# jmg049/Spectrograms

Hardware: AMD Instinct MI355X
Metric: STFT frames/sec (f32, n_fft=1024 hop=256) (higher is better)
Workload: dtype f32

## Files before the change

### spectrograms_amd/csrc/kernels_r32x16.hip

```cpp
#include <type_traits>
#include <utility>

#include "binaural_kind.h"
#include "buffer_ops.h"
#include "fft_inreg.h"
#include "r32x16_layout.h"
#include "sgx_internal.h"

namespace sgx {
namespace {

using namespace inreg;
using namespace r32x16;

typedef int v4i __attribute__((ext_vector_type(4)));
typedef int v2i __attribute__((ext_vector_type(2)));

__device__ __forceinline__ float db_f32(float x) { return __builtin_log2f(x) * 3.01029995663981195f; }

template <int AMP>
__device__ __forceinline__ float amp_f32(float p, float eps) {
    if constexpr (AMP == AMP_MAGNITUDE) return sqrtf(p);
    else if constexpr (AMP == AMP_DB) return db_f32(fmaxf(p, eps));
    else return p;
}
__device__ __forceinline__ float power_of(v2f x) { return __builtin_fmaf(x.x, x.x, x.y * x.y); }

__device__ __forceinline__ unsigned lds_addr(const void *p) { return (unsigned)(size_t)p; }

#ifdef SGX_STAMPS
__device__ unsigned long long g_stamps[32];
#define SGX_STAMP(i)                                                                        \
    do {                                                                                    \
        unsigned long long t_;                                                              \
        __builtin_amdgcn_sched_barrier(0);                                                  \
        asm volatile("s_memtime %0\n\ts_waitcnt lgkmcnt(0)" : "=s"(t_)::"memory");          \
        __builtin_amdgcn_sched_barrier(0);                                                  \
        st_acc[i] += t_ - st_prev;                                                          \
        st_prev = t_;                                                                       \
    } while (0)
#define SGX_STAMP_PARAMS , unsigned long long *st_acc, unsigned long long &st_prev
#define SGX_STAMP_ARGS , st_acc, st_prev
#else
#define SGX_STAMP(i)
#define SGX_STAMP_PARAMS
#define SGX_STAMP_ARGS
#endif

#ifndef SGX_BANDSEG
#define SGX_BANDSEG 0
#endif
#ifndef SGX_BANDTRIP
#define SGX_BANDTRIP 0
#endif
#ifndef SGX_BANDFMA
#define SGX_BANDFMA 0
#endif
#ifndef SGX_BANDPF
#define SGX_BANDPF 0
#endif
#ifndef SGX_ODDHOP
#define SGX_ODDHOP 1
#endif
#ifndef SGX_DMA
#define SGX_DMA 0
#endif
#ifndef SGX_ONEPATH
#define SGX_ONEPATH 1
#endif

template <int OFF>
__device__ __forceinline__ void ds_read64(v2f &d, unsigned addr) {
    asm volatile("ds_read_b64 %0, %1 offset:%2" : "=v"(d) : "v"(addr), "n"(OFF));
}
template <int OFF>
__device__ __forceinline__ void ds_read128(v4f &d, unsigned addr) {
    asm volatile("ds_read_b128 %0, %1 offset:%2" : "=v"(d) : "v"(addr), "n"(OFF));
}
template <int N>
__device__ __forceinline__ void tie8(v2f *d) {
    if constexpr (N >= 0)
        asm volatile("s_waitcnt lgkmcnt(%8)"
                     : "+v"(d[0]), "+v"(d[1]), "+v"(d[2]), "+v"(d[3]), "+v"(d[4]), "+v"(d[5]), "+v"(d[6]), "+v"(d[7])
                     : "n"(N));
    else
        asm volatile("" : "+v"(d[0]), "+v"(d[1]), "+v"(d[2]), "+v"(d[3]), "+v"(d[4]), "+v"(d[5]), "+v"(d[6]), "+v"(d[7]));
}
template <int N>
__device__ __forceinline__ void tie16(v2f (&d)[16]) {
    tie8<N>(&d[0]);
    tie8<-1>(&d[8]);
}
template <bool XSPAD, int N1>
constexpr int col_off() { return N1 * 128 + (XSPAD ? (N1 >> 3) * 128 : 0); }
template <bool XSPAD, int PAR, int... K>
__device__ __forceinline__ void read_cols(v2f (&x)[16], v2f (&w)[16], unsigned xaddr, unsigned waddr, std::integer_sequence<int, K...>) {
    ((ds_read64<col_off<XSPAD, 2 * K + PAR>()>(x[K], xaddr), ds_read64<(2 * K + PAR) * 128>(w[K], waddr)), ...);
}

template <int HOP>
constexpr int p512_off_a(int n1) { return 64 * n1 + (64 * n1 / (8 * HOP)) * 64; }
template <int HOP>
constexpr int p512_off_b(int n1) { return 64 * n1 + 4 * HOP + ((64 * n1 + 4 * HOP) / (8 * HOP)) * 64; }
template <int O0, int O1>
__device__ __forceinline__ void ds_read2x32(v2f &d, unsigned addr) {
    static_assert(O0 >= 0 && O0 < 256 && O1 >= 0 && O1 < 256, "ds_read2_b32: 8-bit dword offsets");
    asm volatile("ds_read2_b32 %0, %1 offset0:%2 offset1:%3" : "=v"(d) : "v"(addr), "n"(O0), "n"(O1));
}
template <int HOP, int PAR, int... K>
__device__ __forceinline__ void read_cols512(v2f (&x)[16], v2f (&w)[16], const unsigned (&base)[8], unsigned waddr, std::integer_sequence<int, K...>) {
    ((ds_read2x32<(p512_off_a<HOP>(2 * K + PAR) - p512_off_a<HOP>((2 * K + PAR) & ~3)) / 4, (p512_off_b<HOP>(2 * K + PAR) - p512_off_a<HOP>((2 * K + PAR) & ~3)) / 4>(
          x[K], base[(2 * K + PAR) >> 2]),
      ds_read64<(2 * K + PAR) * 128>(w[K], waddr)),
     ...);
}

template <int PAR, int... K>
__device__ __forceinline__ void read_cols_odd(v2f (&x)[16], v2f (&w)[16], const unsigned (&base)[4], unsigned waddr, std::integer_sequence<int, K...>) {
    ((ds_read2x32<((2 * K + PAR) & 7) * 32, ((2 * K + PAR) & 7) * 32 + 1>(x[K], base[(2 * K + PAR) >> 3]), ds_read64<(2 * K + PAR) * 128>(w[K], waddr)), ...);
}

template <int PAR, int... K>
__device__ __forceinline__ void read_win(v2f (&w)[16], unsigned waddr, std::integer_sequence<int, K...>) {
    (ds_read64<(2 * K + PAR) * 128>(w[K], waddr), ...);
}

template <int OFF>
__device__ __forceinline__ void dma16_to_lds(__amdgpu_buffer_rsrc_t r, int voff, unsigned lds_base) {
    unsigned keep;
    asm volatile("s_mov_b32 %0, m0\n\ts_mov_b32 m0, %3\n\ts_nop 0\n\tbuffer_load_dwordx4 %1, %2, 0 offen offset:%4 lds\n\ts_mov_b32 m0, %0"
                 : "=&s"(keep)
                 : "v"(voff), "s"(r), "s"(lds_base), "n"(OFF)
                 : "memory");
}
template <bool XSPAD, int R, int ROUNDS>
__device__ __forceinline__ void dma_rounds(__amdgpu_buffer_rsrc_t r, int voff, unsigned xs_base, unsigned wave) {
    if constexpr (R < ROUNDS) {
        const unsigned c0 = R * 256u + wave * 64u;
        dma16_to_lds<0>(r, voff + R * 4096, xs_base + c0 * 16u + (XSPAD ? (c0 >> 6) * 128u : 0u));
        dma_rounds<XSPAD, R + 1, ROUNDS>(r, voff, xs_base, wave);
    }
}

template <bool CONJ>
__device__ __forceinline__ v2f cmul_reg(v2f x, v2f t) {
    const v2f c = x * lo2(t);
    v2f r;
    if constexpr (CONJ) asm("v_pk_fma_f32 %0, %1, %2, %3 op_sel:[1,1,0] op_sel_hi:[0,1,1] neg_hi:[0,1,0]" : "=v"(r) : "v"(x), "v"(t), "v"(c));
    else asm("v_pk_fma_f32 %0, %1, %2, %3 op_sel:[1,1,0] op_sel_hi:[0,1,1] neg_lo:[0,1,0]" : "=v"(r) : "v"(x), "v"(t), "v"(c));
    return r;
}
__device__ __forceinline__ v2f split_tw(v2f D, v2f w) {
    const v2f c = lo2(D) * w;
    v2f r;
    asm("v_pk_fma_f32 %0, %1, %2, %3 op_sel:[1,1,0] op_sel_hi:[1,0,1] neg_lo:[0,1,0]" : "=v"(r) : "v"(D), "v"(w), "v"(c));
    return r;
}

__device__ __forceinline__ void load_tw1(const StftArgs &a, unsigned n2, v2f (&twa)[4], v2f (&twb)[8]) {
    const v2f *t1 = (const v2f *)a.tw1 + n2;
#pragma unroll
    for (int q = 0; q < 4; ++q) twa[q] = t1[16 * 8 * q];
#pragma unroll
    for (int q = 0; q < 8; ++q) twb[q] = t1[16 * q];
}

template <bool P2>
__device__ __forceinline__ void twiddle_store(v2f (&xr)[32], const v2f (&twa)[4], const v2f (&twb)[8], unsigned char *dst) {
#pragma unroll
    for (int k1 = 0; k1 < 32; ++k1) {
        const int qa = k1 >> 3, qb = k1 & 7;
        v2f r = xr[k1];
        if constexpr (P2) {
            if (k1 == 0) r = cmul_reg<true>(r, twa[2]);
        } else {
            if (qb) r = cmulv(r, twb[qb]);
            if (qa) r = cmulv(r, twa[qa]);
        }
#if defined(SGX_ABL_NOEXW)
        asm volatile("" ::"v"(r), "v"(dst));
#elif defined(SGX_ABL_ADDTID)
        asm volatile("ds_write_addtid_b32 %0 offset:%2\n\tds_write_addtid_b32 %1 offset:%3" ::"v"(r.x), "v"(r.y), "n"(k1 * 512), "n"(k1 * 512 + 256) : "memory");
#else
        *(v2f *)(dst + k1 * 128) = r;
#endif
    }
}

__device__ __forceinline__ void read_rows(const unsigned char *exf, unsigned ra, unsigned rb, v2f (&A)[16], v2f (&B)[16]) {
    const v4f *pa = (const v4f *)(exf + ra * 128);
    const v4f *pb = (const v4f *)(exf + rb * 128);
#pragma unroll
    for (int c = 0; c < 8; ++c) {
        const v4f q = pa[c];
        A[2 * c] = (v2f){q.x, q.y};
        A[2 * c + 1] = (v2f){q.z, q.w};
    }
#pragma unroll
    for (int c = 0; c < 8; ++c) {
        const v4f q = pb[c];
        B[2 * c] = (v2f){q.x, q.y};
        B[2 * c + 1] = (v2f){q.z, q.w};
    }
}

struct JobOfs {
    unsigned a1, b1, a2, b2, mid;
};
__device__ __forceinline__ JobOfs job_offsets(unsigned j, unsigned n_frames) {
    const unsigned c1 = j == 0 ? 16u : j, c2 = j == 0 ? 0u : j + 256u;
    return JobOfs{c1 * n_frames, (512u - 224u - c1) * n_frames, c2 * n_frames, (512u - 224u - c2) * n_frames, 256u * n_frames};
}

__device__ __forceinline__ void pass2_twiddle(v2f (&A)[16], v2f (&B)[16], const v2f (&t)[16]) {
#pragma unroll
    for (int n = 1; n < 16; ++n) {
        A[n] = cmul_reg<false>(A[n], t[n]);
        B[n] = cmul_reg<true>(B[n], t[n]);
    }
}

struct PwAddr {
    float *up, *down;
};
template <int MODE, int AMP, bool PWT, bool ROT>
__device__ __forceinline__ void pass2_compute(v2f (&A)[16], v2f (&B)[16], bool j0, float eps, const v4f *tw, __amdgpu_buffer_rsrc_t ro,
                                              unsigned oa1, unsigned ob1, unsigned oa2, unsigned ob2, unsigned omid, unsigned step,
                                              float *pw_c1, float *pw_m1, float *pw_c2, float *pw_m2, float *pw_mid SGX_STAMP_PARAMS) {
    constexpr int R = ROT ? 1 : 0;
    Fft<16, false>::run(A, A);
    Fft<16, false>::run(B, B);
    const v2f a8 = ROT ? B[9] : A[8];
    if (j0) {
        if constexpr (ROT) {
            v2f nA[8], nB[16];
#pragma unroll
            for (int t = 0; t < 8; ++t) nA[t] = B[t + 1];
#pragma unroll
            for (int i = 0; i < 8; ++i) nB[(16 - i) & 15] = A[15 - i];
#pragma unroll
            for (int t = 0; t < 8; ++t) nB[8 - t] = B[(17 - t) & 15];
#pragma unroll
            for (int t = 0; t < 8; ++t) A[8 + t] = nA[t];
#pragma unroll
            for (int i = 0; i < 16; ++i) B[i] = nB[i];
        } else {
            v2f nA[16], nB[8];
#pragma unroll
            for (int i = 0; i < 8; ++i) { nA[i] = B[i]; nA[8 + i] = A[i]; }
            nB[7] = A[0];
#pragma unroll
            for (int t = 1; t < 8; ++t) nB[7 - t] = A[16 - t];
#pragma unroll
            for (int i = 0; i < 16; ++i) A[i] = nA[i];
#pragma unroll
            for (int i = 0; i < 8; ++i) B[i] = nB[i];
        }
        asm volatile("" ::: "memory");
    }
    SGX_STAMP(9);
    constexpr int PSTEP = MODE == OUT_BINAURAL ? 32 * 16 * 2 : PWT ? 32 * 16 : 32;
    auto emit = [&](unsigned voff, unsigned soff, float *pwp, v2f X, bool conj) {
#ifdef SGX_ABL_NOSTORE
        asm volatile("" ::"v"(X), "v"(voff));
        return;
#endif
        if constexpr (MODE == OUT_COMPLEX) {
            const v2f V = conj ? (v2f){X.x, -X.y} : X;
            __builtin_amdgcn_raw_buffer_store_b64(__builtin_bit_cast(v2i, V), ro, (int)voff, (int)soff, 0);
        } else if constexpr (MODE == OUT_MEL) {
#ifdef SGX_ABL_NOPW
            asm volatile("" ::"v"(X), "v"(pwp));
            return;
#endif
            *pwp = AMP == AMP_MAG_IN ? sqrtf(power_of(X)) : power_of(X);
        } else if constexpr (MODE == OUT_BINAURAL) {
            *(v2f *)pwp = conj ? (v2f){X.x, -X.y} : X;
        } else {
            __builtin_amdgcn_raw_buffer_store_b32(__builtin_bit_cast(int, amp_f32<AMP>(power_of(X), eps)), ro, (int)voff, (int)soff, 0);
        }
    };
    auto twi = [&](int i) {
        const v4f q = tw[i >> 1];
        return (i & 1) ? (v2f){q.z, q.w} : (v2f){q.x, q.y};
    };
    auto split = [&](v2f P, v2f Q, v2f w, v2f &X, v2f &Y) {
        const v2f E = pfma(Q, (v2f){1.f, -1.f}, P);
        const v2f D = pfma(Q, (v2f){-1.f, 1.f}, P);
        const v2f T = split_tw(D, w);
        X = E + T;
        Y = E - T;
    };
#pragma unroll
    for (int i = 0; i < 8; ++i) {
        v2f X, Y;
        split(A[i], B[(15 + R - i) & 15], twi(i), X, Y);
        emit(oa1, i * step, pw_c1 + i * PSTEP, X, false);
        emit(ob1, (7 - i) * step, pw_m1 + (7 - i) * PSTEP, Y, true);
    }
#pragma unroll
    for (int t = 0; t < 8; ++t) {
        v2f X, Y;
        split(A[8 + t], B[7 + R - t], twi(8 + t), X, Y);
        emit(oa2, t * step, pw_c2 + t * PSTEP, X, false);
        emit(ob2, (7 - t) * step, pw_m2 + (7 - t) * PSTEP, Y, true);
    }
    if (j0) emit(omid, 0u, pw_mid, a8 * (v2f){2.f, -2.f}, false);
    SGX_STAMP(10);
}

constexpr unsigned kP512Step = 16u * 64u;
template <int MODE, int AMP, bool PACK = false>
__device__ __forceinline__ void pass2_pair512(v2f (&A)[16], v2f (&B)[16], bool j0, float eps, __amdgpu_buffer_rsrc_t ro, unsigned vfull1,
                                              unsigned vhalf1, unsigned vfull2, unsigned vhalf2, unsigned vfullm, unsigned vhalfm, unsigned step,
                                              float *pw1, float *pw2, float *pwm) {
    Fft<16, false>::run(A, A);
    Fft<16, false>::run(B, B);
    const v2f a8 = A[8];
    if (j0) {
        v2f nA[16], nB[8];
#pragma unroll
        for (int i = 0; i < 8; ++i) { nA[i] = B[i]; nA[8 + i] = A[i]; }
        nB[7] = A[0];
#pragma unroll
        for (int t = 1; t < 8; ++t) nB[7 - t] = A[16 - t];
#pragma unroll
        for (int i = 0; i < 16; ++i) A[i] = nA[i];
#pragma unroll
        for (int i = 0; i < 8; ++i) B[i] = nB[i];
        asm volatile("" ::: "memory");
    }
    auto emit = [&](unsigned vfull, unsigned vhalf, int soff, v2f Xa, v2f Xb, bool conj, float *pwp) {
        if constexpr (MODE == OUT_MEL) {
            const float pa = power_of(Xa), pb = power_of(Xb);
            *(v2f *)pwp = AMP == AMP_MAG_IN ? (v2f){sqrtf(pa), sqrtf(pb)} : (v2f){pa, pb};
        } else if constexpr (MODE == OUT_COMPLEX) {
            const float sg = conj ? -1.f : 1.f;
            const v4f V = (v4f){Xa.x, sg * Xa.y, Xb.x, sg * Xb.y};
            if constexpr (PACK) {
                __builtin_amdgcn_raw_buffer_store_b64(__builtin_bit_cast(v2i, (v2f){V.x, V.y}), ro, (int)vfull, soff, 0);
                __builtin_amdgcn_raw_buffer_store_b64(__builtin_bit_cast(v2i, (v2f){V.z, V.w}), ro, (int)vhalf, soff, 0);
            } else {
                __builtin_amdgcn_raw_buffer_store_b128(__builtin_bit_cast(v4i, V), ro, (int)vfull + soff, 0, 0);
                __builtin_amdgcn_raw_buffer_store_b64(__builtin_bit_cast(v2i, (v2f){V.x, V.y}), ro, (int)vhalf, soff, 0);
            }
        } else {
            const v2f V = (v2f){amp_f32<AMP>(power_of(Xa), eps), amp_f32<AMP>(power_of(Xb), eps)};
            if constexpr (PACK) {
                const float va = V.x, vb = V.y;
                __builtin_amdgcn_raw_buffer_store_b32(__builtin_bit_cast(int, va), ro, (int)vfull, soff, 0);
                __builtin_amdgcn_raw_buffer_store_b32(__builtin_bit_cast(int, vb), ro, (int)vhalf, soff, 0);
            } else {
                __builtin_amdgcn_raw_buffer_store_b64(__builtin_bit_cast(v2i, V), ro, (int)vfull, soff, 0);
                __builtin_amdgcn_raw_buffer_store_b32(__builtin_bit_cast(int, V.x), ro, (int)vhalf, soff, 0);
            }
        }
    };
    auto pair = [&](v2f P, v2f Q, v2f &Xa, v2f &Xb) {
        Xa = pfma(Q, (v2f){1.f, -1.f}, P);
        const v2f D = pfma(Q, (v2f){-1.f, 1.f}, P);
        Xb = (v2f){D.y, -D.x};
    };
#pragma unroll
    for (int i = 0; i < 8; ++i) {
        v2f Xa, Xb;
        pair(A[i], B[15 - i], Xa, Xb);
        emit(vfull1, vhalf1, i * (int)step, Xa, Xb, false, pw1 + i * kP512Step);
    }
#pragma unroll
    for (int t = 0; t < 8; ++t) {
        v2f Xa, Xb;
        pair(A[8 + t], B[7 - t], Xa, Xb);
        if (j0) emit(vfull2 + t * step, vhalf2 + t * step, 0, Xa, Xb, false, pw2 + t * kP512Step);
        else emit(vfull2 + (7 - t) * step, vhalf2 + (7 - t) * step, 0, Xa, Xb, true, pw2 + (7 - t) * kP512Step);
    }
    if (j0) emit(vfullm, vhalfm, 0, (v2f){2.f * a8.x, 0.f}, (v2f){2.f * a8.y, 0.f}, false, pwm);
}

template <int AMP>
__device__ __forceinline__ void mel_tile_csr(const StftArgs &a, const float *pwall, unsigned b, unsigned f0, unsigned nf,
                                             float eps, unsigned t, unsigned nthreads) {
    const float *val = (const float *)a.mel_val;
    float *o = (float *)a.out + ((size_t)b * a.n_out) * a.n_frames + f0;
    for (unsigned idx = t; idx < 16u * a.n_mels; idx += nthreads) {
        const unsigned ff = idx & 15u, mm = idx >> 4;
        float acc = 0.0f;
// ... 233 lines not shown
    }
}

template <int STEPS>
constexpr int mfcc_row() { return (STEPS / 4) % 2 ? STEPS : STEPS + 4; }
template <int STEPS>
__device__ __forceinline__ void mfcc_tile(const StftArgs &a, const float *mq, const float *frag, unsigned mt, unsigned b, unsigned f0, unsigned nf,
                                          unsigned lane) {
    static_assert(STEPS % 4 == 0, "chain lengths are whole 16-byte reads");
    constexpr int RL = mfcc_row<STEPS>();
    const unsigned n = lane & 15u, q = lane >> 4;
    const bool mine = mt < a.mfcc_mtiles;
    v4acc acc = {0.f, 0.f, 0.f, 0.f};
    if (mine) {
        const v4f *pa = (const v4f *)(frag + ((size_t)mt * 64u + lane) * RL);
        const v4f *pb = (const v4f *)(mq + (q * 16u + n) * RL);
        v4f wa[STEPS / 4], vb[STEPS / 4];
#pragma unroll
        for (int g = 0; g < STEPS / 4; ++g) { wa[g] = pa[g]; vb[g] = pb[g]; }
#pragma unroll
        for (int g = 0; g < STEPS / 4; ++g) {
            acc = __builtin_amdgcn_mfma_f32_16x16x4f32(wa[g].x, vb[g].x, acc, 0, 0, 0);
            acc = __builtin_amdgcn_mfma_f32_16x16x4f32(wa[g].y, vb[g].y, acc, 0, 0, 0);
            acc = __builtin_amdgcn_mfma_f32_16x16x4f32(wa[g].z, vb[g].z, acc, 0, 0, 0);
            acc = __builtin_amdgcn_mfma_f32_16x16x4f32(wa[g].w, vb[g].w, acc, 0, 0, 0);
        }
    }
    const float *lift = frag + (size_t)a.mfcc_mtiles * 64u * RL;
    constexpr unsigned kDrop = 0x80000000u;
    const unsigned rows = a.n_mfcc - a.mfcc_skip;
    const unsigned obytes = (rows * a.n_frames - f0) * 4u;
    const __amdgpu_buffer_rsrc_t ro = make_rsrc((const float *)a.out + (size_t)b * rows * a.n_frames + f0, obytes);
    const unsigned mtr = mine ? mt : 0u;
#pragma unroll
    for (int r = 0; r < 4; ++r) {
        const unsigned c = 16u * mtr + 4u * q + r;
        const bool ok = mine && c >= a.mfcc_skip && c < a.n_mfcc && n < nf;
        __builtin_amdgcn_raw_buffer_store_b32(__builtin_bit_cast(int, acc[r] * lift[min(c, a.n_mfcc - 1u)]), ro,
                                              (int)(ok ? ((c - a.mfcc_skip) * a.n_frames + n) * 4u : kDrop), 0, 0);
    }
}

__host__ __device__ constexpr unsigned pwt512_index(unsigned k, unsigned f) { return (k >> 1) * 64u + (f >> 1) * 4u + (k & 1u) * 2u + (f & 1u); }
template <int AMP>
__device__ __forceinline__ void mel_tile_sched512(const StftArgs &a, const float *pwT, const unsigned *sched, unsigned b, unsigned f0,
                                                  unsigned nf, float eps, unsigned tid) {
    const unsigned wave = __builtin_amdgcn_readfirstlane(tid >> 6), lane = tid & 63u, slot = lane >> 4, fp = lane & 15u;
    const unsigned obytes = (a.n_out * a.n_frames - f0) * 4u;
    const __amdgpu_buffer_rsrc_t ro = make_rsrc((const float *)a.out + (size_t)b * a.n_out * a.n_frames + f0, obytes);
    constexpr unsigned kDrop = 0x80000000u;
    const unsigned fo0 = 2u * fp < nf ? 8u * fp : kDrop, fo1 = 2u * fp + 1u < nf ? 8u * fp + 4u : kDrop;
    const uint4 *info = (const uint4 *)(sched + kSchedHdr) + wave * 8u + slot;
    uint4 ca = info[0], cb = info[4];
#pragma unroll
    for (unsigned seg = 0; seg < (unsigned)kSchedSegs; ++seg) {
        const uint4 na = info[(seg + 1u) * 32u], nb = info[(seg + 1u) * 32u + 4u];
        const unsigned L = __builtin_amdgcn_readfirstlane(ca.x);
        const v4f *wa = (const v4f *)((const float *)sched + ca.y), *wb = (const v4f *)((const float *)sched + cb.y);
        const v4f *pa = (const v4f *)(pwT + (ca.z >> 1) * 64u) + fp, *pb = (const v4f *)(pwT + (cb.z >> 1) * 64u) + fp;
        v2f acca = {0.0f, 0.0f}, accb = {0.0f, 0.0f};
        for (unsigned t = 0; t < L; t += 4u) {
            const v4f w4a = wa[t >> 2], a0 = pa[(t >> 1) * 16u], a1 = pa[(t >> 1) * 16u + 16u];
            const v4f w4b = wb[t >> 2], b0 = pb[(t >> 1) * 16u], b1 = pb[(t >> 1) * 16u + 16u];
            acca = mul_add_unfused(w4a.x, (v2f){a0.x, a0.y}, acca);
            accb = mul_add_unfused(w4b.x, (v2f){b0.x, b0.y}, accb);
            acca = mul_add_unfused(w4a.y, (v2f){a0.z, a0.w}, acca);
            accb = mul_add_unfused(w4b.y, (v2f){b0.z, b0.w}, accb);
            acca = mul_add_unfused(w4a.z, (v2f){a1.x, a1.y}, acca);
            accb = mul_add_unfused(w4b.z, (v2f){b1.x, b1.y}, accb);
            acca = mul_add_unfused(w4a.w, (v2f){a1.z, a1.w}, acca);
            accb = mul_add_unfused(w4b.w, (v2f){b1.z, b1.w}, accb);
        }
        const bool ha = ca.w != 0xffffffffu, hb = cb.w != 0xffffffffu;
        const unsigned boa = ca.w * a.n_frames * 4u, bob = cb.w * a.n_frames * 4u;
        __builtin_amdgcn_raw_buffer_store_b32(__builtin_bit_cast(int, amp_f32<AMP>(acca.x, eps)), ro, (int)((ha && fo0 != kDrop) ? boa + fo0 : kDrop), 0, 0);
        __builtin_amdgcn_raw_buffer_store_b32(__builtin_bit_cast(int, amp_f32<AMP>(acca.y, eps)), ro, (int)((ha && fo1 != kDrop) ? boa + fo1 : kDrop), 0, 0);
        __builtin_amdgcn_raw_buffer_store_b32(__builtin_bit_cast(int, amp_f32<AMP>(accb.x, eps)), ro, (int)((hb && fo0 != kDrop) ? bob + fo0 : kDrop), 0, 0);
        __builtin_amdgcn_raw_buffer_store_b32(__builtin_bit_cast(int, amp_f32<AMP>(accb.y, eps)), ro, (int)((hb && fo1 != kDrop) ? bob + fo1 : kDrop), 0, 0);
        ca = na;
        cb = nb;
    }
}

template <int KIND>
__device__ __forceinline__ void binaural_tile(const StftArgs &a, const unsigned char *smem_all, unsigned b, unsigned f0, unsigned nf) {
    binaural::KindConst<float> c;
    c.pi = 3.14159265358979323846f;
    c.two_pi = 2.0f * c.pi;
    c.bw = (float)a.bin_bw;
    c.power = a.bin_power;
    c.wrapped = a.bin_wrapped;
    const v2f *L = (const v2f *)smem_all, *R = (const v2f *)(smem_all + kExBytes);
    float *out = (float *)a.out + ((size_t)b * a.bin_count) * a.n_frames + f0;
    for (unsigned i = threadIdx.x; i < a.bin_count * 16u; i += 512u) {
        const unsigned r = i >> 4, f = i & 15u, k = a.bin_start + r;
        const v2f l = L[k * 16u + f], q = R[k * 16u + f];
        const float v = binaural::binaural_value<float, KIND>(l.x, l.y, q.x, q.y, k, c);
        if (f < nf) out[(size_t)r * a.n_frames + f] = v;
    }
}

template <int MODE, int AMP, int ROUNDS, bool WIDE, bool XSPAD, bool PWT, int HOP512 = 0, bool PACK = false, int MSTEPS = 0>
__global__ __launch_bounds__(512, 2) void k_r32x16(StftArgs a, unsigned per_xcd, unsigned total, unsigned slots) {
    constexpr bool MFCC = MSTEPS != 0;
    static_assert(!MFCC || (PWT && AMP == AMP_DB && HOP512 == 0 && !PACK), "fused MFCC epilogue: Mel-dB on the schedule, n_fft 1024, one-signal tiles");
    constexpr bool P512 = HOP512 != 0;
    constexpr bool BIN = MODE == OUT_BINAURAL;
    static_assert(!BIN || (!WIDE && !PWT && !P512 && !PACK && !MFCC), "binaural: one-signal n_fft 1024 tiles, per-half pass 2");
    constexpr unsigned HS = BIN ? 1u : 2u;
    static_assert(!PACK || (ROUNDS == 0 && !WIDE && !XSPAD && (HOP512 == 0 ? (MODE != OUT_MEL || PWT) : MODE != OUT_MEL)),
                  "PACK: direct loads, one-half tiles; n_fft 1024: scheduled band stage, n_fft 512: per-bin outputs");
    constexpr unsigned SS512 = 8u * HOP512;
    static_assert(!P512 || PACK || (HOP512 % 4 == 0 && ROUNDS * 256 * 4 >= 31 * HOP512 + 512), "P512: 16-byte chunks, the whole tile staged");
    static_assert(!WIDE || MODE != OUT_MEL, "wide pass 2 needs a per-bin output");
    static_assert(!PWT || MODE == OUT_MEL, "PWT is a filterbank layout");
    static_assert(!P512 || (!WIDE && !XSPAD && (ROUNDS > 0 || PACK) && (PWT == (MODE == OUT_MEL))), "P512: staged samples (PACK: per-lane loads), scheduled band stage");
    constexpr bool DMA = SGX_DMA != 0 && PWT && ROUNDS > 0 && !P512;
    constexpr unsigned FPT = P512 ? 32u : 16u;
    constexpr unsigned NB = P512 ? 257u : 513u;
    extern __shared__ __attribute__((aligned(16))) unsigned char smem_all[];
    const unsigned half = __builtin_amdgcn_readfirstlane(threadIdx.x >> 8);
    const unsigned tid = threadIdx.x & 255u;
    constexpr bool H256M = HOP512 == 256 && MODE == OUT_MEL && !PACK;
    constexpr unsigned EXB = H256M ? (unsigned)kExBytesH256 : (unsigned)kExBytes, POFF = H256M ? (unsigned)kOutOffH256 : (unsigned)kOutOff;
    unsigned char *smem = smem_all + half * EXB;
    unsigned char *tabs = smem_all + 2 * EXB;
    if (threadIdx.x < 256u) ((v4f *)(tabs + kWinOff))[threadIdx.x] = ((const v4f *)a.window)[threadIdx.x];
    if (threadIdx.x < 256u) {
        const unsigned jj = threadIdx.x >> 4, ii = threadIdx.x & 15u;
        const v4f q = ((const v4f *)a.tw2)[jj * 17u + ii];
        *(v2f *)(tabs + kTw2Off + jj * kTw2Stride + ii * 8u) = (v2f){q.x, q.y};
        *(v2f *)(tabs + kTrOff + jj * 128u + ii * 8u) = ((const v2f *)a.tw1)[(jj == 0u ? 16u : jj) * 16u + ii];
    }
    unsigned *sched = (unsigned *)(tabs + kMelOff);
    if constexpr (PWT)
        for (unsigned i = threadIdx.x; i < a.mel_sched_words; i += 512u) sched[i] = a.mel_sched[i];
    float *mfrag = (float *)(tabs + kMelOff) + ((a.mel_sched_words + 3u) & ~3u);
    if constexpr (MFCC)
        for (unsigned i = threadIdx.x; i < a.mfcc_frag_words; i += 512u) mfrag[i] = ((const float *)a.mfcc_frag)[i];

    const unsigned xcd = blockIdx.x & 7u, slot = blockIdx.x >> 3;
    const unsigned lo = xcd * per_xcd;
    const unsigned hi = min(lo + per_xcd, total);
    unsigned wid = lo + slot * HS + (BIN ? 0u : half);
    unsigned lead = lo + slot * HS;

    const unsigned p1f = tid >> 4, n2 = tid & 15u;
    const unsigned lane = tid & 63u;
    const unsigned wv_ = WIDE ? threadIdx.x >> 6 : tid >> 6;
    const unsigned jq = WIDE ? lane >> 5 : lane >> 4, p2f = WIDE ? lane & 31u : lane & 15u;
    const unsigned j = wv_ + (WIDE ? 8u : 4u) * jq;
    constexpr bool TWP2 = !P512 && MODE != OUT_MEL;
    constexpr bool TRLDS = TWP2 && ROUNDS == 0 && !WIDE;
    const unsigned ra = j == 0 ? (TWP2 ? 16u : 0u) : j, rb = j == 0 ? (TWP2 ? 0u : 16u) : 32u - j;
    const float eps = (float)a.eps;
    constexpr unsigned ES = MODE == OUT_COMPLEX ? 8u : 4u;
    const JobOfs jo = job_offsets(j, a.n_frames);
    const unsigned step = 32u * a.n_frames * ES;
    const v4f *twj = (const v4f *)(tabs + kTw2Off + j * kTw2Stride);
    v2f twa[4], twb[8], tr[16];
    if constexpr (!TWP2) {
        load_tw1(a, n2, twa, twb);
    } else {
        twa[2] = ((const v2f *)a.tw1)[16 * 16 + n2];
        if constexpr (!TRLDS)
#pragma unroll
            for (int q = 0; q < 16; ++q) tr[q] = ((const v2f *)a.tw1)[ra * 16u + q];
    }

    constexpr int NCR = ROUNDS > 0 ? ROUNDS : 1;
    v4f creg[NCR];
    v2f xd[ROUNDS > 0 ? 1 : 32];
    const unsigned chunks = XSPAD ? 1216u : P512 ? (31u * HOP512 + 512u + 3u) >> 2 : (15u * a.hop + 1024u + 3u) >> 2;
    const unsigned hop = XSPAD ? 256u : (P512 && !PACK) ? (unsigned)HOP512 : a.hop;
    const unsigned row_bytes = (unsigned)a.n_samples * 4u;
    auto load_tile = [&](unsigned w) {
        const unsigned b = w / a.tiles, tile = w - b * a.tiles;
        const unsigned f0 = tile * FPT;
        const __amdgpu_buffer_rsrc_t rx = make_rsrc((const float *)(BIN && half ? a.x2 : a.x) + (size_t)b * a.sample_stride, row_bytes);
        const int tile_lo = (int)(f0 * hop) - (int)a.pad;
        const bool interior = tile_lo >= 0 && (unsigned)tile_lo + (FPT - 1u) * hop + (P512 ? 512u : 1024u) <= (unsigned)a.n_samples;
        if constexpr (ROUNDS > 0) {
#ifdef SGX_ABL_NOGLOAD
            for (int r = 0; r < ROUNDS; ++r) creg[r] = (v4f){(float)w, 1.f, 2.f, (float)r};
            return;
#endif
            const int vo = (tile_lo + 4 * (int)tid) * 4;
            if constexpr (DMA) {
                dma_rounds<XSPAD, 0, ROUNDS>(rx, vo, lds_addr(smem), __builtin_amdgcn_readfirstlane(tid >> 6));
                return;
            }
            if (SGX_ONEPATH || interior || P512) {
#pragma unroll
                for (int r = 0; r < ROUNDS; ++r)
                    if (SGX_ONEPATH || XSPAD || P512 || r * 256u + tid < chunks) creg[r] = __builtin_bit_cast(v4f, __builtin_amdgcn_raw_buffer_load_b128(rx, vo + r * 4096, 0, 0));
            } else {
#pragma unroll
                for (int r = 0; r < ROUNDS; ++r) {
                    v4i c;
#pragma unroll
                    for (int e = 0; e < 4; ++e) c[e] = __builtin_amdgcn_raw_buffer_load_b32(rx, vo + r * 4096 + 4 * e, 0, 0);
                    creg[r] = __builtin_bit_cast(v4f, c);
                }
            }
        } else if constexpr (PACK && P512) {
            const __amdgpu_buffer_rsrc_t rall = make_rsrc(a.x, a.x_bytes);
            const unsigned ns = (unsigned)a.n_samples, PP = (a.n_frames + 1u) >> 1;
            const unsigned q = w * 16u + p1f;
            const bool live = q < a.gframes;
            const unsigned bq = live ? q / PP : 0u, pr = q - bq * PP;
            const int sA = (int)(2u * pr * hop) - (int)a.pad + (int)n2, sB = sA + (int)hop;
            const unsigned row = bq * (unsigned)a.sample_stride;
#pragma unroll
            for (int n1 = 0; n1 < 32; ++n1) {
                const int ia = sA + 16 * n1, ib = sB + 16 * n1;
                const int va = __builtin_amdgcn_raw_buffer_load_b32(rall, (live && (unsigned)ia < ns) ? (int)((row + (unsigned)ia) * 4u) : (int)0xfffffff0u, 0, 0);
                const int vb = __builtin_amdgcn_raw_buffer_load_b32(rall, (live && (unsigned)ib < ns) ? (int)((row + (unsigned)ib) * 4u) : (int)0xfffffff0u, 0, 0);
                xd[n1] = (v2f){__builtin_bit_cast(float, va), __builtin_bit_cast(float, vb)};
            }
        } else if constexpr (PACK) {
            const unsigned g = w * 16u + p1f;
            const bool live = g < a.gframes;
            const unsigned bq = live ? g / a.n_frames : 0u, fq = g - bq * a.n_frames;
            const __amdgpu_buffer_rsrc_t rall = make_rsrc(a.x, a.x_bytes);
            const int s0 = (int)(fq * hop) - (int)a.pad + 2 * (int)n2;
            const unsigned rowo = bq * (unsigned)a.sample_stride;
            const unsigned ns = (unsigned)a.n_samples;
#pragma unroll
            for (int n1 = 0; n1 < 32; ++n1) {
                const int sidx = s0 + 32 * n1;
                const bool in0 = live && (unsigned)sidx < ns;
                v2f v = __builtin_bit_cast(v2f, __builtin_amdgcn_raw_buffer_load_b64(rall, in0 ? (int)((rowo + (unsigned)sidx) * 4u) : (int)0xfffffff0u, 0, 0));
                if ((unsigned)(sidx + 1) >= ns) v.y = 0.0f;
                xd[n1] = v;
            }
        } else {
            const int vo = ((int)(p1f * hop) + tile_lo + 2 * (int)n2) * 4;
            if (SGX_ONEPATH || interior) {
#pragma unroll
                for (int n1 = 0; n1 < 32; ++n1) xd[n1] = __builtin_bit_cast(v2f, __builtin_amdgcn_raw_buffer_load_b64(rx, vo + n1 * 128, 0, 0));
#if SGX_ODDHOP
                if (a.hop & 1u) {
                    const float x0 = __builtin_bit_cast(float, __builtin_amdgcn_raw_buffer_load_b32(rx, 0, 0, 0));
                    const int s0 = (int)(p1f * hop) + tile_lo + 2 * (int)n2;
#pragma unroll
                    for (int n1 = 0; n1 < 32; ++n1)
                        if (s0 + 32 * n1 == -1) xd[n1].y = x0;
                }
#endif
            } else {
#pragma unroll
                for (int n1 = 0; n1 < 32; ++n1) {
                    v2i c;
                    c.x = __builtin_amdgcn_raw_buffer_load_b32(rx, vo + n1 * 128, 0, 0);
                    c.y = __builtin_amdgcn_raw_buffer_load_b32(rx, vo + n1 * 128 + 4, 0, 0);
                    xd[n1] = __builtin_bit_cast(v2f, c);
                }
            }
        }
    };

    if (wid >= hi) wid = lead;
    if (lead < hi) load_tile(wid);
    if constexpr (DMA) asm volatile("s_waitcnt vmcnt(0)" ::: "memory");
    __syncthreads();

    const unsigned xaddr = lds_addr(smem) + p1f * hop * 4u + n2 * 8u + (XSPAD ? p1f * 128u : 0u);
    const unsigned waddr = lds_addr(tabs + kWinOff) + n2 * 8u;

#ifdef SGX_SKEW
    if (MODE == OUT_MEL && half == 1u)
        for (unsigned q = 0; q < SGX_SKEW; ++q) __syncthreads();
#endif
#ifndef SGX_STAGGER
#define SGX_STAGGER 4u
#endif
    if constexpr (MODE != OUT_MEL) {
        for (unsigned q = 0; q < (blockIdx.x >> 3) * SGX_STAGGER; ++q) __builtin_amdgcn_s_sleep(1);
        __syncthreads();
    }
#ifdef SGX_PRIO
    if (half == SGX_PRIO - 1u) __builtin_amdgcn_s_setprio(1);
#endif
#ifdef SGX_STAMPS
    unsigned long long st_acc[16] = {0}, st_prev;
    asm volatile("s_memtime %0\n\ts_waitcnt lgkmcnt(0)" : "=s"(st_prev)::"memory");
#endif
    const unsigned mfcc_mt = (((threadIdx.x & 255u) >> 6) + 4u - half) & 3u;
    float *const mfl = (float *)(smem + kOutOff) - 64 * mfcc_row<MFCC ? MSTEPS : 4>();
    unsigned pvb = 0, pvf0 = 0, pvnf = 0;
    static_assert(!MFCC || kOutOff - 256 * mfcc_row<MFCC ? MSTEPS : 4>() >= 22912, "Mel-dB tile above the staged samples");
    while (lead < hi) {
        const unsigned PP = (a.n_frames + 1u) >> 1;
        const unsigned b = PACK ? (P512 ? wid * 16u / PP : wid * 16u / a.n_frames) : wid / a.tiles, tile = wid - b * a.tiles;
        const unsigned f0 = PACK ? wid * 16u - b * a.n_frames : tile * FPT;
        const unsigned nf = PACK ? min(16u, a.gframes - wid * 16u) : min(FPT, a.n_frames - f0);
        v2f xr[32];
        {
            v2f e[16], o[16], we[16], wo[16];
            if constexpr (ROUNDS > 0) {
                if constexpr (DMA) {
                    asm volatile("s_waitcnt vmcnt(%0)" ::"n"(2 * kSchedSegs) : "memory");
                } else {
#pragma unroll
                for (int r = 0; r < ROUNDS; ++r) {
                    const unsigned c = r * 256u + tid;
                    if (SGX_ONEPATH || XSPAD || P512 || c < chunks) *(v4f *)(smem + c * 16u + (XSPAD ? (c >> 6) * 128u : P512 ? (c * 16u / (P512 ? SS512 : 1u)) * 64u : 0u)) = creg[r];
                }
                }
                SGX_STAMP(0);
                __syncthreads();
                SGX_STAMP(1);
                if constexpr (MFCC) mfcc_tile<MFCC ? MSTEPS : 4>(a, mfl, mfrag, mfcc_mt, pvb, pvf0, pvnf, tid & 63u);
                if constexpr (HOP512 == 256) {
                    const float *pa = (const float *)(smem + p1f * (SS512 + 64u) + n2 * 4u);
#pragma unroll
                    for (int k = 0; k < 16; ++k) {
                        e[k] = (v2f){pa[p512_off_a<256>(2 * k) / 4], pa[p512_off_b<256>(2 * k) / 4]};
                        o[k] = (v2f){pa[p512_off_a<256>(2 * k + 1) / 4], pa[p512_off_b<256>(2 * k + 1) / 4]};
                    }
                    read_win<0>(we, waddr, std::make_integer_sequence<int, 16>{});
                    read_win<1>(wo, waddr, std::make_integer_sequence<int, 16>{});
                    tie16<0>(e);
                    tie16<-1>(o);
                    tie16<-1>(we);
                    tie16<-1>(wo);
                } else if constexpr (P512) {
                    unsigned base[8];
#pragma unroll
                    for (int q = 0; q < 8; ++q) base[q] = lds_addr(smem) + p1f * (SS512 + 64u) + n2 * 4u + (unsigned)p512_off_a<P512 ? HOP512 : 128>(4 * q);
                    read_cols512<P512 ? HOP512 : 128, 0>(e, we, base, waddr, std::make_integer_sequence<int, 16>{});
                    read_cols512<P512 ? HOP512 : 128, 1>(o, wo, base, waddr, std::make_integer_sequence<int, 16>{});
                    tie16<15>(e);
                    tie16<-1>(we);
                } else {
                if (SGX_ODDHOP && !XSPAD && (a.hop & 1u)) {
                    const unsigned base[4] = {xaddr, xaddr + 1024u, xaddr + 2048u, xaddr + 3072u};
                    read_cols_odd<0>(e, we, base, waddr, std::make_integer_sequence<int, 16>{});
                    read_cols_odd<1>(o, wo, base, waddr, std::make_integer_sequence<int, 16>{});
                } else {
                read_cols<XSPAD, 0>(e, we, xaddr, waddr, std::make_integer_sequence<int, 16>{});
                read_cols<XSPAD, 1>(o, wo, xaddr, waddr, std::make_integer_sequence<int, 16>{});
                }
                tie16<15>(e);
                tie16<-1>(we);
                }
            } else {
                const v2f *w2 = (const v2f *)(tabs + kWinOff) + n2;
#pragma unroll
                for (int k = 0; k < 16; ++k) {
                    e[k] = xd[2 * k];
                    o[k] = xd[2 * k + 1];
                    we[k] = w2[32 * k];
                    wo[k] = w2[32 * k + 16];
                }
            }
            Fft<16, true>::run(e, we);
            if constexpr (ROUNDS > 0) {
                tie16<0>(o);
                tie16<-1>(wo);
            }
            Fft<16, true>::run(o, wo);
            Comb<32, 0, v2f>::run(xr, e, o);
        }
        SGX_STAMP(2);
        if constexpr (ROUNDS > 0 || MFCC) __syncthreads();
        SGX_STAMP(3);
#ifdef SGX_ABL_ADDTID
        {
            const unsigned m0v = __builtin_amdgcn_readfirstlane(lds_addr(smem) + (tid >> 6) * 16384u);
            asm volatile("s_mov_b32 m0, %0\n\ts_nop 0" ::"s"(m0v) : "memory");
        }
#endif
        twiddle_store<TWP2>(xr, twa, twb, smem + p1f * kFS + n2 * 8);
        SGX_STAMP(4);
        unsigned next = lead + slots * HS + (BIN ? 0u : half);
        if (next >= hi) next -= BIN ? 0u : half;
        if constexpr (!DMA)
            if (lead + slots * HS < hi) load_tile(next);
        SGX_STAMP(5);
        __syncthreads();
        SGX_STAMP(6);
        constexpr bool ALLSTORE = MODE != OUT_MEL;
        unsigned p2b = b, p2ofs, p2ex;
        if constexpr (WIDE) {
            const unsigned w1 = lead + 1u < hi ? lead + 1u : lead;
            const unsigned b0 = lead / a.tiles, f00 = (lead - b0 * a.tiles) * 16u;
            const unsigned b1 = w1 / a.tiles, f01 = (w1 - b1 * a.tiles) * 16u;
            const unsigned nf0 = min(16u, a.n_frames - f00), nf1 = min(16u, a.n_frames - f01);
            const bool second = p2f >= 16u && w1 != lead;
            const unsigned fle = min(p2f & 15u, (second ? nf1 : nf0) - 1u);
            p2ex = (second ? 16u : 0u) + fle;
            p2ofs = (second ? f01 : f00) + fle + ((second && b1 != b0) ? 513u * a.n_frames : 0u);
            p2b = b0;
        } else if constexpr (P512) {
            p2ex = p2f;
            p2ofs = f0 + 2u * p2f;
        } else if constexpr (PACK) {
            const unsigned p2f_eff = ALLSTORE ? min(p2f, nf - 1u) : p2f;
            const unsigned fl = f0 + p2f_eff, bq = fl / a.n_frames;
            p2ex = p2f_eff;
            p2ofs = bq * NB * a.n_frames + (fl - bq * a.n_frames);
        } else {
            const unsigned p2f_eff = ALLSTORE ? min(p2f, nf - 1u) : p2f;
            p2ex = p2f_eff;
            p2ofs = f0 + p2f_eff;
        }
        v2f A[16], B[16];
        read_rows((WIDE ? smem_all : smem) + p2ex * kFS, ra, rb, A, B);
        if constexpr (TRLDS) {
            const v4f *tq = (const v4f *)(tabs + kTrOff + j * 128u);
#pragma unroll
            for (int q = 0; q < 8; ++q) {
                const v4f t2 = tq[q];
                tr[2 * q] = (v2f){t2.x, t2.y};
                tr[2 * q + 1] = (v2f){t2.z, t2.w};
            }
        }
        if constexpr (TWP2) pass2_twiddle(A, B, tr);
        SGX_STAMP(7);
        __syncthreads();
        SGX_STAMP(8);
        if constexpr (DMA)
            if (lead + slots * HS < hi) load_tile(next);
        float *pwf = (float *)(smem + (PWT ? POFF : 0u));
        if constexpr (MODE == OUT_MEL) {
            if constexpr (P512) {
                for (unsigned i = tid; i < 11u * 32u; i += 256u) pwf[pwt512_index(257u + (i >> 5), i & 31u)] = 0.0f;
            } else if constexpr (PWT) {
                if (tid < 176u) pwf[pwt_index(513u + (tid >> 4), tid & 15u)] = 0.0f;
            } else {
                if (tid < 48u) pwf[(tid / 3u) * kPS + 513u + tid % 3u] = 0.0f;
            }
        }
        if constexpr (BIN) {
            const unsigned c1 = j == 0 ? 16u : j, c2 = j == 0 ? 0u : j + 256u;
            auto slot_of = [&](unsigned k) { return (float *)smem + (k * 16u + p2f) * 2u; };
            pass2_compute<MODE, AMP, false, TWP2>(A, B, j == 0, eps, twj, make_rsrc(a.out, 0u), 0u, 0u, 0u, 0u, 0u, 0u, slot_of(c1),
                                            slot_of(512u - 224u - c1), slot_of(c2), slot_of(512u - 224u - c2), slot_of(256u) SGX_STAMP_ARGS);
            __syncthreads();
            binaural_tile<AMP>(a, smem_all, b, f0, nf);
            __syncthreads();
        } else if constexpr (P512 && PACK) {
            constexpr unsigned kDrop = 0x80000000u;
            const __amdgpu_buffer_rsrc_t ro = make_rsrc((unsigned char *)a.out + (size_t)b * NB * a.n_frames * ES, min(17u, a.batch - b) * NB * a.n_frames * ES);
            const unsigned c1 = j == 0 ? 16u : j, r2 = j == 0 ? 0u : 32u - j;
            const unsigned q = wid * 16u + p2f, bq = q / PP, pr = q - bq * PP;
            const unsigned oA = p2f < nf ? ((bq - b) * NB * a.n_frames + 2u * pr) * ES : kDrop;
            const unsigned oB = (p2f < nf && 2u * pr + 1u < a.n_frames) ? oA + ES : kDrop;
            auto at = [&](unsigned base, unsigned row) { return base == kDrop ? kDrop : base + row * a.n_frames * ES; };
            pass2_pair512<MODE, AMP, true>(A, B, j == 0, eps, ro, at(oA, c1), at(oB, c1), at(oA, r2), at(oB, r2), at(oA, 256u), at(oB, 256u), step,
                                           nullptr, nullptr, nullptr);
        } else if constexpr (P512) {
            constexpr unsigned kDrop = 0x80000000u;
            const __amdgpu_buffer_rsrc_t ro = make_rsrc((unsigned char *)a.out + (size_t)b * NB * a.n_frames * ES, NB * a.n_frames * ES);
            const unsigned c1 = j == 0 ? 16u : j, r2 = j == 0 ? 0u : 32u - j;
            const unsigned nv = 2u * p2f + 1u < nf ? 2u : 2u * p2f < nf ? 1u : 0u;
            const unsigned o1 = (c1 * a.n_frames + p2ofs) * ES, o2 = (r2 * a.n_frames + p2ofs) * ES, om = (256u * a.n_frames + p2ofs) * ES;
            float *pws = pwf + 4u * p2f;
            pass2_pair512<MODE, AMP>(A, B, j == 0, eps, ro, nv == 2u ? o1 : kDrop, nv == 1u ? o1 : kDrop, nv == 2u ? o2 : kDrop,
                                     nv == 1u ? o2 : kDrop, nv == 2u ? om : kDrop, nv == 1u ? om : kDrop, step, pws + pwt512_index(c1, 0u),
                                     pws + pwt512_index(r2, 0u), pws + pwt512_index(256u, 0u));
        } else if (ALLSTORE || p2f < nf) {
            const unsigned c1 = j == 0 ? 16u : j, c2 = j == 0 ? 0u : j + 256u;
            const unsigned long long obytes = (unsigned long long)min(PACK ? 17u : 2u, a.batch - p2b) * 513ull * a.n_frames * ES;
            const __amdgpu_buffer_rsrc_t ro = make_rsrc((unsigned char *)a.out + (size_t)p2b * 513u * a.n_frames * ES, (unsigned)obytes);
            {
                auto slot_of = [&](unsigned k) { return pwf + (PWT ? pwt_index(k, p2f) : p2f * kPS + k); };
                pass2_compute<MODE, AMP, PWT, TWP2>(A, B, j == 0, eps, twj, ro, (jo.a1 + p2ofs) * ES, (jo.b1 + p2ofs) * ES, (jo.a2 + p2ofs) * ES,
                                                     (jo.b2 + p2ofs) * ES, (jo.mid + p2ofs) * ES, step, slot_of(c1), slot_of(512u - 224u - c1),
                                                     slot_of(c2), slot_of(512u - 224u - c2), slot_of(256u) SGX_STAMP_ARGS);
            }
        }
        if constexpr (MODE == OUT_MEL) {
            __syncthreads();
            SGX_STAMP(11);
#ifdef SGX_ABL_NOMEL
            if (a.n_mels == 12345u)
#endif
            if constexpr (P512) mel_tile_sched512<AMP>(a, pwf, sched, b, f0, nf, eps, tid);
            else if constexpr (MFCC) {
                mel_tile_sched<AMP, false, mfcc_row<MFCC ? MSTEPS : 4>()>(a, pwf, sched, b, f0, nf, eps, tid, mfl SGX_STAMP_ARGS);
                if constexpr (ROUNDS > 0) {
                    pvb = b; pvf0 = f0; pvnf = nf;
                } else {
                    __syncthreads();
                    mfcc_tile<MFCC ? MSTEPS : 4>(a, mfl, mfrag, mfcc_mt, b, f0, nf, tid & 63u);
                }
            }
            else if constexpr (PWT) mel_tile_sched<AMP, PACK>(a, pwf, sched, b, f0, nf, eps, tid, nullptr SGX_STAMP_ARGS);
            else if (a.mm_frag) map_tile_mfma<AMP>(a, pwf, b, f0, nf, eps, tid, 2u * half);
            else mel_tile_csr<AMP>(a, pwf, b, f0, nf, eps, tid, 256u);
            if constexpr (!PWT) __syncthreads();
        }
        SGX_STAMP(14);
        wid = next;
        lead += slots * HS;
#ifdef SGX_STAMPS
        st_acc[15] += 1;
#endif
    }
    if constexpr (MFCC && ROUNDS > 0) {
        __syncthreads();
        mfcc_tile<MFCC ? MSTEPS : 4>(a, mfl, mfrag, mfcc_mt, pvb, pvf0, pvnf, tid & 63u);
    }
#ifdef SGX_SKEW
    if (MODE == OUT_MEL && half == 0u)
        for (unsigned q = 0; q < SGX_SKEW; ++q) __syncthreads();
#endif
#ifdef SGX_STAMPS
    if ((threadIdx.x & 63u) == 0) {
        for (int q = 0; q < 16; ++q) atomicAdd(&g_stamps[q], st_acc[q]);
        atomicAdd(&g_stamps[16], 1ull);
    }
#endif
}

static bool want_pack(const StftArgs &a, bool mel, bool pwt) {
    if (a.mfcc_frag) return false;
    const bool p512 = a.n_fft == 512u;
    const bool unlisted512 = p512 && !(a.hop == 64u || a.hop == 128u || a.hop == 160u || a.hop == 256u);
    if ((a.n_fft != 1024u && !p512) || (a.batch < 2u && !unlisted512) || (mel && (!pwt || p512)) || (a.hop & 1u)) return false;
    const unsigned long long slots = (unsigned long long)a.tiles * a.ft, g = (unsigned long long)a.batch * a.n_frames;
    const unsigned long long used = p512 ? 2ull * ((a.n_frames + 1ull) / 2ull) : a.n_frames;
    if ((slots - used) * 4ull < slots && !unlisted512) return false;
    if (g >= 0x7fffffffull || (unsigned long long)a.batch * a.sample_stride * 4ull >= 0xfffffff0ull) return false;
    return (a.ft + 1ull) * (a.n_fft / 2u + 1ull) * a.n_frames * 8ull < 0x7fffffffull;
}

template <int MODE, int AMP>
hipError_t launch_variant(const StftArgs &a0, hipStream_t s) {
    StftArgs a = a0;
    const bool pack = want_pack(a, MODE == OUT_MEL, MODE == OUT_MEL && a.mel_sched != nullptr);
// ... 161 lines not shown
```

Measured before the change: 1.455 billion.

## Overlap odd-half FFT and fused combine-store with the LDS barrier

```diff
diff --git a/spectrograms_amd/csrc/kernels_r32x16.hip b/spectrograms_amd/csrc/kernels_r32x16.hip
--- a/spectrograms_amd/csrc/kernels_r32x16.hip
+++ b/spectrograms_amd/csrc/kernels_r32x16.hip
@@ -65,6 +65,9 @@
 #ifndef SGX_DMA
 #define SGX_DMA 0
 #endif
+#ifndef SGX_OVL
+#define SGX_OVL 1
+#endif
 #ifndef SGX_ONEPATH
 #define SGX_ONEPATH 1
 #endif
@@ -95,7 +98,12 @@
 constexpr int col_off() { return N1 * 128 + (XSPAD ? (N1 >> 3) * 128 : 0); }
 template <bool XSPAD, int PAR, int... K>
 __device__ __forceinline__ void read_cols(v2f (&x)[16], v2f (&w)[16], unsigned xaddr, unsigned waddr, std::integer_sequence<int, K...>) {
+#ifdef SGX_ABL_NOWIN
+    ((ds_read64<col_off<XSPAD, 2 * K + PAR>()>(x[K], xaddr), w[K] = (v2f){0.5f, 0.25f}), ...);
+    asm volatile("" ::"v"(waddr));
+#else
     ((ds_read64<col_off<XSPAD, 2 * K + PAR>()>(x[K], xaddr), ds_read64<(2 * K + PAR) * 128>(w[K], waddr)), ...);
+#endif
 }
 
 template <int HOP>
@@ -122,7 +130,16 @@
 
 template <int PAR, int... K>
 __device__ __forceinline__ void read_win(v2f (&w)[16], unsigned waddr, std::integer_sequence<int, K...>) {
+#ifdef SGX_ABL_NOWIN
+    ((w[K] = (v2f){0.5f, 0.25f}), ...);
+    asm volatile("" ::"v"(waddr));
+#else
     (ds_read64<(2 * K + PAR) * 128>(w[K], waddr), ...);
+#endif
+}
+template <int OFF>
+__device__ __forceinline__ void ds_write64(unsigned addr, v2f d) {
+    asm volatile("ds_write_b64 %0, %1 offset:%2" ::"v"(addr), "v"(d), "n"(OFF) : "memory");
 }
 
 template <int OFF>
@@ -185,6 +202,24 @@
         *(v2f *)(dst + k1 * 128) = r;
 #endif
     }
+}
+
+template <int... K>
+__device__ __forceinline__ void comb_store(const v2f (&e)[16], const v2f (&o)[16], v2f t16, unsigned dst, std::integer_sequence<int, K...>) {
+    auto one = [&](auto kc) {
+        constexpr int k1 = decltype(kc)::value;
+        v2f x0, x1;
+        bfly<32, k1, v2f>(e[k1], o[k1], x0, x1);
+        if constexpr (k1 == 0) x0 = cmul_reg<true>(x0, t16);
+#if defined(SGX_ABL_NOEXW)
+        asm volatile("" ::"v"(x0), "v"(x1), "v"(dst));
+#else
+        ds_write64<k1 * 128>(dst, x0);
+        ds_write64<(k1 + 16) * 128>(dst, x1);
+#endif
+        __builtin_amdgcn_sched_barrier(0);
+    };
+    (one(std::integral_constant<int, K>{}), ...);
 }
 
 __device__ __forceinline__ void read_rows(const unsigned char *exf, unsigned ra, unsigned rb, v2f (&A)[16], v2f (&B)[16]) {
@@ -231,7 +266,11 @@
     Fft<16, false>::run(A, A);
     Fft<16, false>::run(B, B);
     const v2f a8 = ROT ? B[9] : A[8];
+#ifdef SGX_ABL_NOJ0
+    if (false) {
+#else
     if (j0) {
+#endif
         if constexpr (ROT) {
             v2f nA[8], nB[16];
 #pragma unroll
@@ -771,6 +810,7 @@
     const unsigned j = wv_ + (WIDE ? 8u : 4u) * jq;
     constexpr bool TWP2 = !P512 && MODE != OUT_MEL;
     constexpr bool TRLDS = TWP2 && ROUNDS == 0 && !WIDE;
+    constexpr bool OVL = SGX_OVL != 0 && MODE == OUT_LINEAR && !P512 && ROUNDS > 0;
     const unsigned ra = j == 0 ? (TWP2 ? 16u : 0u) : j, rb = j == 0 ? (TWP2 ? 0u : 16u) : 32u - j;
     const float eps = (float)a.eps;
     constexpr unsigned ES = MODE == OUT_COMPLEX ? 8u : 4u;
@@ -979,25 +1019,37 @@
                 tie16<0>(o);
                 tie16<-1>(wo);
             }
+            if constexpr (OVL) {
+                SGX_STAMP(2);
+                __syncthreads();
+                __builtin_amdgcn_sched_barrier(0);
+                SGX_STAMP(3);
+                Fft<16, true>::run(o, wo);
+                comb_store(e, o, twa[2], lds_addr(smem + p1f * kFS + n2 * 8), std::make_integer_sequence<int, 16>{});
+            } else {
             Fft<16, true>::run(o, wo);
             Comb<32, 0, v2f>::run(xr, e, o);
-        }
+            }
+        }
+        if constexpr (!OVL) {
         SGX_STAMP(2);
         if constexpr (ROUNDS > 0 || MFCC) __syncthreads();
         SGX_STAMP(3);
+        }
 #ifdef SGX_ABL_ADDTID
         {
             const unsigned m0v = __builtin_amdgcn_readfirstlane(lds_addr(smem) + (tid >> 6) * 16384u);
             asm volatile("s_mov_b32 m0, %0\n\ts_nop 0" ::"s"(m0v) : "memory");
         }
 #endif
-        twiddle_store<TWP2>(xr, twa, twb, smem + p1f * kFS + n2 * 8);
+        if constexpr (!OVL) twiddle_store<TWP2>(xr, twa, twb, smem + p1f * kFS + n2 * 8);
         SGX_STAMP(4);
         unsigned next = lead + slots * HS + (BIN ? 0u : half);
         if (next >= hi) next -= BIN ? 0u : half;
         if constexpr (!DMA)
             if (lead + slots * HS < hi) load_tile(next);
         SGX_STAMP(5);
+        if constexpr (OVL) asm volatile("s_waitcnt lgkmcnt(0)" ::: "memory");
         __syncthreads();
         SGX_STAMP(6);
         constexpr bool ALLSTORE = MODE != OUT_MEL;
```

After: 1.461 billion (median of 3 runs). Within noise of the previous version (+0.4%).
